# rhmes/point-cloud-compression

Hardware: AMD Instinct MI355X
Metric: points/sec compress+decompress (ModelNet40-shaped 8192 K=256) (higher is better)
Workload: dtype f32 (operands split into two scaled fp16 pieces of 22-23 bits together, three fp16-MFMA products per fp32 product, fp32 accumulate); 1 GPU; IPDAE K=256 d=16 L=7, 8192-pt CAD-like synthetic clouds (configs[1]); distinct_clouds_per_gpu=1024, points_per_cloud=8192, patches_per_cloud=64, octree_mode=reference, weights=seeded random, matmul=f16x2

## Files before the change

### point-cloud-compression_amd/csrc/encoder_fused_h2.hip

```cpp
#include <math.h>
#include <stdlib.h>

#include "blobs.h"
#include "common.h"
#include "mfma_chain.h"

#ifndef FH_CHUNK
#define FH_CHUNK PN_H2_CHUNK
#endif
static_assert(FH_CHUNK % 8 == 0 && ((PN_H2_STREAM_FRAGS + FH_CHUNK - 1) / FH_CHUNK) * FH_CHUNK <= PN_H2_STREAM_CHUNKS * PN_H2_CHUNK, "the padded stream must cover the last chunk");
#ifndef FH_SA_MG
#define FH_SA_MG 2
#endif
#ifndef FH_NB
#define FH_NB 2
#endif
#ifndef FH_MG
#define FH_MG 2
#endif
#ifndef FH_READER
#define FH_READER 1
#endif
#ifndef FH_FIFO
#define FH_FIFO 8
#endif
#ifndef FH_FIFO2
#define FH_FIFO2 8
#endif
#define FH_STAGE_STRIDE 132
#define FH_STAGE_WAVE (16 * FH_STAGE_STRIDE)

__host__ __device__ inline size_t fh_region_bytes()
{
    const size_t ring = (size_t)FH_NB * FH_CHUNK * 1024, stage = (size_t)8 * FH_STAGE_WAVE * 4;
    return ring > stage ? ring : stage;
}
__host__ __device__ inline size_t fh_lds_bytes(int K)
{
    return (size_t)(ENC_H2_SA_W1_FRAGS + ENC_H2_SA_W2_FRAGS) * 1024 + (64 + 128 + ENC_H2_PN_BIAS_FLOATS) * 4 + (size_t)K * 12 + (size_t)K * 32 +
           fh_region_bytes() + 8 * 16 * 4 + 32 + 16;
}

template <bool NT2>
__global__ __launch_bounds__(512, 1) void sa_pn_forward_h2_kernel(const float *__restrict__ x, int npatches, int K, const float *__restrict__ blob,
                                                                  const float *__restrict__ h2, int d, float spread, float half_spread,
                                                                  float *__restrict__ latent_raw, float *__restrict__ latent,
                                                                  float *__restrict__ latent_q, const unsigned char *__restrict__ nbr_tab,
                                                                  const int *__restrict__ uniq, const int *__restrict__ n_uniq)
{
    extern __shared__ __attribute__((aligned(16))) unsigned char smem[];
    f32x4 *sw1 = (f32x4 *)smem;
    f32x4 *sw2 = sw1 + ENC_H2_SA_W1_FRAGS * 64;
    float *sb1 = (float *)(sw2 + ENC_H2_SA_W2_FRAGS * 64);
    float *sb2 = sb1 + 64;
    float *spb = sb2 + 128;
    float *sx = spb + ENC_H2_PN_BIAS_FLOATS;
    unsigned short *nbr16 = (unsigned short *)(sx + 3 * K);
    unsigned char *region = (unsigned char *)(nbr16 + 16 * K);
    f32x4 *swt = (f32x4 *)region;
    float *stage_all = (float *)region;
    float (*smax)[16] = (float (*)[16])(region + fh_region_bytes());
    int *sa_next = (int *)(region + fh_region_bytes() + 8 * 16 * 4);
    unsigned *srmax = (unsigned *)(sa_next + 8);

    const int ntiles = K >> 4;
    const int wu = __builtin_amdgcn_readfirstlane((int)threadIdx.x >> 6);
    auto fresh_lane = []() {
        int l = (int)__builtin_amdgcn_mbcnt_hi(~0u, __builtin_amdgcn_mbcnt_lo(~0u, 0u));
        asm volatile("" : "+v"(l));
        return l;
    };
    auto meta = [&](int i) { return __uint_as_float(__builtin_amdgcn_readfirstlane(__float_as_uint(opaque_uniform(h2)[ENC_H2_META + i]))); };
    {
        const int tid0 = threadIdx.x;
        const f32x4 *gw = (const f32x4 *)(h2 + ENC_H2_SA_W);
        for (int i = tid0; i < (ENC_H2_SA_W1_FRAGS + ENC_H2_SA_W2_FRAGS) * 64; i += 512) sw1[i] = gw[i];
        if (tid0 == 0) *srmax = 0u;
    }
    __syncthreads();
  const int nlist = uniq ? *n_uniq : npatches;
  for (int slot = blockIdx.x; slot < nlist; slot += gridDim.x) {
    const size_t P = uniq ? (size_t)uniq[slot] : (size_t)slot;
    const int lane = fresh_lane(), tid = wu * 64 + lane;
    const float *xp = x + P * (size_t)K * 3;
    {
        unsigned m = 0u;
        for (int i = tid; i < 3 * K; i += 512) m = max(m, __float_as_uint(xp[i]) & 0x7FFFFFFFu);
#pragma unroll
        for (int o = 32; o >= 1; o >>= 1) m = max(m, (unsigned)__shfl_xor((int)m, o));
        if (lane == 0) atomicMax(srmax, m);
    }
    if (tid < 8) sa_next[tid] = 0;
    {
        const uint4 *tab = (const uint4 *)nbr_tab + P * (size_t)K * (K <= 256 ? 1 : 2);
        if (K <= 256) {
            for (int i = tid; i < K; i += 512) {
                const uint4 v = tab[i];
                const unsigned b[4] = {v.x, v.y, v.z, v.w};
                unsigned wd[8];
#pragma unroll
                for (int q = 0; q < 4; ++q) {
                    wd[2 * q] = (b[q] & 0xFFu) | ((b[q] & 0xFF00u) << 8);
                    wd[2 * q + 1] = ((b[q] >> 16) & 0xFFu) | ((b[q] >> 8) & 0xFF0000u);
                }
                ((uint4 *)nbr16)[2 * i] = make_uint4(wd[0], wd[1], wd[2], wd[3]);
                ((uint4 *)nbr16)[2 * i + 1] = make_uint4(wd[4], wd[5], wd[6], wd[7]);
            }
        } else {
            for (int i = tid; i < 2 * K; i += 512) ((uint4 *)nbr16)[i] = tab[i];
        }
    }
    __syncthreads();
    const int rexp = (int)((unsigned)__builtin_amdgcn_readfirstlane((int)*srmax) >> 23) - 127;
    const float s = rexp >= 0 ? __uint_as_float((unsigned)(126 - rexp) << 23) : 1.0f;
    const float inv_s = rexp >= 0 ? __uint_as_float((unsigned)(128 + rexp) << 23) : 1.0f;
    for (int i = tid; i < 3 * K; i += 512) sx[i] = xp[i] * s;
    if (tid < 64) sb1[tid] = h2[ENC_H2_SA_B1 + tid] * s;
    if (tid < 128) sb2[tid] = h2[ENC_H2_SA_B2 + tid] * s;
    for (int i = tid; i < ENC_H2_PN_BIAS_FLOATS; i += 512) spb[i] = h2[ENC_H2_PN_B0 + i] * s;
    __syncthreads();
    if (tid == 0) *srmax = 0u;

    const f32x4 zero4 = {0.f, 0.f, 0.f, 0.f};
    if (lane < 16) smax[wu][lane] = -INFINITY;

    auto sa_and_handover = [&](int it, f16x8 (&i0p)[1][5][2], bool &valid) {
        const int tile = it * 8 + wu;
        valid = tile < ntiles;
        const int p0 = (valid ? tile : 0) * 16;
        int lane = fresh_lane();
        int g = lane >> 4, n = lane & 15;
        const float rho0 = meta(H2E_RHO0), rho1 = meta(H2E_RHO1), inv2 = meta(H2E_INV2);
        const float w0a = blob[ENC_SA_W0B0 + 4 * n + g], w0b = blob[ENC_SA_W0B0 + 4 * (16 + n) + g];

        const int pass_base = it * 128;
        const int units = ((K - pass_base < 128 ? K - pass_base : 128) + 1) >> 1;
        for (;;) {
            int unit = 0;
            if (lane == 0) unit = atomicAdd(&sa_next[it & 7], 1);
            unit = __builtin_amdgcn_readfirstlane(unit);
            if (unit >= units) break;
            const int i0 = pass_base + 2 * unit;
            f32x4 h0[2][2];
#pragma unroll
            for (int nt = 0; nt < 2; ++nt) {
                const int i = i0 + nt;
                const int j = nbr16[i * 16 + n];
                const float rel = g < 3 ? __fsub_rn(sx[3 * j + g], sx[3 * i + g]) : s;
                h0[nt][0] = relu4(mfma16(w0a, rel, zero4));
                h0[nt][1] = relu4(mfma16(w0b, rel, zero4));
            }
            f32x4 a1[2][4];
#pragma unroll
            for (int mt = 0; mt < 4; ++mt) a1[0][mt] = a1[1][mt] = *(const f32x4 *)(sb1 + 16 * mt + 4 * g);
            f32x4 a2[2][8];
#pragma unroll
            for (int mt = 0; mt < 8; ++mt) a2[0][mt] = a2[1][mt] = zero4;
            f16x8 i1[2][1][2];
#pragma unroll
            for (int nt = 0; nt < 2; ++nt) h2_split8(h0[nt][0], h0[nt][1], rho0, i1[nt][0]);
            dense_h2<1, 4, 2>(sw1, lane, i1, a1);
            f16x8 i2[2][2][2];
#pragma unroll
            for (int nt = 0; nt < 2; ++nt)
#pragma unroll
                for (int t = 0; t < 2; ++t) h2_split8(relu4(a1[nt][2 * t]), relu4(a1[nt][2 * t + 1]), rho1, i2[nt][t]);
            dense_h2<2, 8, 2, true, FH_SA_MG>(sw2, lane, i2, a2);
#pragma unroll
            for (int nt = 0; nt < 2; ++nt) {
                float mx[2];
                max16_of_8_transposed_tiles(a2[nt], mx);
#pragma unroll
                for (int s2 = 0; s2 < 2; ++s2) {
                    const int ch = 16 * (2 * g + s2) + n;
                    stage_all[(i0 + nt - pass_base) * FH_STAGE_STRIDE + ch] = fmaxf(__fadd_rn(__fmul_rn(mx[s2], inv2), sb2[ch]), 0.f);
                }
            }
        }

        __syncthreads();
        lane = fresh_lane();
        g = lane >> 4; n = lane & 15;
        {
            const float rho_in = meta(H2E_RHO_IN);
            f32x4 in[9];
            const float *stage_t = stage_all + (valid ? p0 - pass_base : 0) * FH_STAGE_STRIDE;
#pragma unroll
            for (int kt = 0; kt < 8; ++kt) in[kt] = *(const f32x4 *)(stage_t + n * FH_STAGE_STRIDE + 16 * kt + 4 * g);
            const int p = p0 + n;
            in[8][0] = g == 0 ? sx[3 * p] : 0.f;
            in[8][1] = g == 0 ? sx[3 * p + 1] : 0.f;
            in[8][2] = g == 0 ? sx[3 * p + 2] : 0.f;
            in[8][3] = 0.f;
#pragma unroll
            for (int t = 0; t < 4; ++t) h2_split8(in[2 * t], in[2 * t + 1], rho_in, i0p[0][t]);
            h2_split8(in[8], zero4, rho_in, i0p[0][4]);
        }
        __syncthreads();
    };

    const int passes = (ntiles + 7) / 8;
    if constexpr (!NT2) {
      for (int it = 0; it < passes; ++it) {
        f16x8 i0p[1][5][2];
        bool valid;
        sa_and_handover(it, i0p, valid);
        const int lane = fresh_lane();
        const int g = lane >> 4, n = lane & 15;
        const float rho_p1 = meta(H2E_RHO_P1), rho_p2 = meta(H2E_RHO_P2), rho_p3 = meta(H2E_RHO_P3);
        WStreamT<FH_CHUNK, FH_NB, 8> ws{opaque_uniform(h2) + ENC_H2_PN_STREAM, swt, (PN_H2_STREAM_FRAGS + FH_CHUNK - 1) / FH_CHUNK, lane, wu, false};
        ws.prologue();
        int f = 0;
#if FH_READER
        H2Reader<FH_FIFO, PN_H2_STREAM_FRAGS, decltype(ws)> rd(ws);
        rd.start();
#define FH_DENSE(KT, MT, in, acc) dense_h2_rd<KT, MT, 1>(rd, f, in, acc)
#else
#define FH_DENSE(KT, MT, in, acc) dense_h2_stream<KT, MT, 1, decltype(ws), FH_MG>(ws, f, in, acc)
#endif
        f32x4 a0[1][8];
#pragma unroll
        for (int mt = 0; mt < 8; ++mt) a0[0][mt] = *(const f32x4 *)(spb + 16 * mt + 4 * g);
        FH_DENSE(5, 8, i0p, a0);
        f16x8 p1[8][1][1][2];
        {
            f32x4 a1p[1][16];
            f16x8 i1p[1][4][2];
#pragma unroll
            for (int t = 0; t < 4; ++t) h2_split8(relu4(a0[0][2 * t]), relu4(a0[0][2 * t + 1]), rho_p1, i1p[0][t]);
#pragma unroll
            for (int mt = 0; mt < 16; ++mt) a1p[0][mt] = *(const f32x4 *)(spb + 128 + 16 * mt + 4 * g);
            FH_DENSE(4, 16, i1p, a1p);
#pragma unroll
            for (int kt = 0; kt < 8; ++kt) h2_split8(relu4(a1p[0][2 * kt]), relu4(a1p[0][2 * kt + 1]), rho_p2, p1[kt][0][0]);
        }
        f32x4 a3[1][1];
        a3[0][0] = *(const f32x4 *)(spb + 128 + 256 + 512 + 4 * g);
#pragma clang loop unroll(full)
        for (int h = 0; h < 2; ++h) {
            f32x4 a2p[1][16];
#pragma unroll
            for (int mt = 0; mt < 16; ++mt) a2p[0][mt] = *(const f32x4 *)(spb + 128 + 256 + 16 * (16 * h + mt) + 4 * g);
#pragma clang loop unroll(full)
            for (int kt = 0; kt < 8; ++kt) FH_DENSE(1, 16, p1[kt], a2p);
#pragma clang loop unroll(full)
            for (int kt = 0; kt < 8; ++kt) {
                f16x8 pl[1][1][2];
                h2_split8(relu4(a2p[0][2 * kt]), relu4(a2p[0][2 * kt + 1]), rho_p3, pl[0][0]);
                FH_DENSE(1, 1, pl, a3);
            }
        }
#undef FH_DENSE
        ws.drain();
        if (valid) {
#pragma unroll
            for (int r = 0; r < 4; ++r) {
                const float v = row16_max(a3[0][0][r]);
                if (n == 0) smax[wu][4 * g + r] = fmaxf(smax[wu][4 * g + r], v);
            }
        }
        __syncthreads();
      }
    } else {
      for (int rnd = 0; rnd < passes / 2; ++rnd) {
        f16x8 i1p[2][4][2];
#pragma clang loop unroll(full)
        for (int hf = 0; hf < 2; ++hf) {
            f16x8 i0p[1][5][2];
            bool valid;
            sa_and_handover(2 * rnd + hf, i0p, valid);
            const int lane = fresh_lane();
            const int g = lane >> 4;
            const float rho_p1 = meta(H2E_RHO_P1);
            WStreamT<FH_CHUNK, FH_NB, 8> ws0{opaque_uniform(h2) + ENC_H2_PN_STREAM2, swt, PN_H2_S2_L0_FRAGS / FH_CHUNK, lane, wu, false};
            ws0.prologue();
            int f = 0;
            H2Reader<FH_FIFO2, 80, decltype(ws0)> rd0(ws0);
            rd0.start();
            f32x4 a0[1][8];
#pragma unroll
            for (int mt = 0; mt < 8; ++mt) a0[0][mt] = *(const f32x4 *)(spb + 16 * mt + 4 * g);
            dense_h2_rd<5, 8, 1>(rd0, f, i0p, a0);
#pragma unroll
            for (int t = 0; t < 4; ++t) h2_split8(relu4(a0[0][2 * t]), relu4(a0[0][2 * t + 1]), rho_p1, i1p[hf][t]);
            ws0.drain();
            __syncthreads();
        }
        const int lane = fresh_lane();
        const int g = lane >> 4, n = lane & 15;
        const float rho_p2 = meta(H2E_RHO_P2), rho_p3 = meta(H2E_RHO_P3);
        WStreamT<FH_CHUNK, FH_NB, 8> ws{opaque_uniform(h2) + ENC_H2_PN_STREAM2 + (size_t)PN_H2_S2_L0_FRAGS * 256, swt, PN_H2_S2_MAIN_FRAGS / FH_CHUNK, lane, wu, false};
        ws.prologue();
        int f = 0;
        H2Reader<FH_FIFO2, PN_H2_S2_MAIN_FRAGS, decltype(ws)> rd(ws);
        rd.start();
        f16x8 p1[8][2][1][2];
        {
            f32x4 a1p[2][16];
#pragma unroll
            for (int mt = 0; mt < 16; ++mt) a1p[0][mt] = a1p[1][mt] = *(const f32x4 *)(spb + 128 + 16 * mt + 4 * g);
            dense_h2_rd<4, 16, 2>(rd, f, i1p, a1p);
#pragma unroll
            for (int kt = 0; kt < 8; ++kt)
#pragma unroll
                for (int nt = 0; nt < 2; ++nt) h2_split8(relu4(a1p[nt][2 * kt]), relu4(a1p[nt][2 * kt + 1]), rho_p2, p1[kt][nt][0]);
        }
        f32x4 a3[2][1];
        a3[0][0] = a3[1][0] = *(const f32x4 *)(spb + 128 + 256 + 512 + 4 * g);
#pragma clang loop unroll(full)
        for (int e = 0; e < 8; ++e) {
            f32x4 a2p[2][4];
#pragma unroll
            for (int mt = 0; mt < 4; ++mt) a2p[0][mt] = a2p[1][mt] = *(const f32x4 *)(spb + 128 + 256 + 16 * (4 * e + mt) + 4 * g);
#pragma clang loop unroll(full)
            for (int kt = 0; kt < 8; ++kt) dense_h2_rd<1, 4, 2>(rd, f, p1[kt], a2p);
#pragma clang loop unroll(full)
            for (int t = 0; t < 2; ++t) {
                f16x8 pl[2][1][2];
#pragma unroll
                for (int nt = 0; nt < 2; ++nt) h2_split8(relu4(a2p[nt][2 * t]), relu4(a2p[nt][2 * t + 1]), rho_p3, pl[nt][0]);
                dense_h2_rd<1, 1, 2>(rd, f, pl, a3);
            }
        }
        ws.drain();
#pragma unroll
        for (int nt = 0; nt < 2; ++nt)
#pragma unroll
            for (int r = 0; r < 4; ++r) {
                const float v = row16_max(a3[nt][0][r]);
                if (n == 0) smax[wu][4 * g + r] = fmaxf(smax[wu][4 * g + r], v);
            }
        __syncthreads();
      }
    }
    __syncthreads();
    if (tid < 16 && tid < d) {
        const float inv_out = meta(H2E_INV_OUT);
        float m = smax[0][tid];
#pragma unroll
        for (int k8 = 1; k8 < 8; ++k8) m = fmaxf(m, smax[k8][tid]);
        m = __fmul_rn(__fmul_rn(m, inv_out), inv_s);
        const float sg = 1.0f / (1.0f + expf(-m));
        const float y = __fsub_rn(__fmul_rn(sg, spread), half_spread);
        latent_raw[P * d + tid] = m;
        latent[P * d + tid] = y;
        latent_q[P * d + tid] = rintf(y);
    }
    __syncthreads();
  }
}

extern "C" int pccx_ae_encode_h2_fused_ok(int K)
{
    return (K >= 16 && K <= 1024 && K % 16 == 0 && fh_lds_bytes(K) <= (size_t)160 * 1024) ? 1 : 0;
}

extern "C" size_t pccx_ae_encode_h2_workspace_bytes(int P, int K) { return pccx_patch_knn16_bytes(P, K); }
extern "C" int pccx_ae_encode_h2_tables(const float *patches, int P, int K, const float *enc_blob, const float *h2_blob, int d, int L,
                                        float *latent_raw, float *latent, float *latent_q, const void *workspace, void *stream);

extern "C" int pccx_ae_encode_h2_ws(const float *patches, int P, int K, const float *enc_blob, const float *h2_blob, int d, int L,
                                    float *latent_raw, float *latent, float *latent_q, void *workspace, void *stream)
{
    if (P == 0) return PCCX_OK;
    PCCX_CHECK_ARG(patches && workspace, "pccx_ae_encode_h2_ws: null pointer");
    PCCX_CHECK_ARG(P >= 0 && pccx_ae_encode_h2_fused_ok(K), "pccx_ae_encode_h2_ws: K=%d does not fit the fused kernel (pccx_ae_encode_h2_fused_ok)", K);
    const int rc = pccx_patch_knn16(patches, P, K, workspace, stream);
    if (rc != PCCX_OK) return rc;
    return pccx_ae_encode_h2_tables(patches, P, K, enc_blob, h2_blob, d, L, latent_raw, latent, latent_q, workspace, stream);
}

extern "C" int pccx_ae_encode_h2_tables_list(const float *patches, int P, int K, const float *enc_blob, const float *h2_blob, int d, int L,
                                             float *latent_raw, float *latent, float *latent_q, const void *workspace, const int32_t *uniq,
                                             const int32_t *n_uniq, void *stream)
{
    if (P == 0) return PCCX_OK;
    PCCX_CHECK_ARG(patches && enc_blob && h2_blob && latent_raw && latent && latent_q && workspace, "pccx_ae_encode_h2_tables: null pointer");
    PCCX_CHECK_ARG(P >= 0 && pccx_ae_encode_h2_fused_ok(K), "pccx_ae_encode_h2_tables: K=%d does not fit the fused kernel (pccx_ae_encode_h2_fused_ok)", K);
    PCCX_CHECK_ARG(d >= 1 && d <= 16 && L >= 1, "pccx_ae_encode_h2_tables: unsupported d=%d L=%d", d, L);
    PCCX_CHECK_ARG(!uniq == !n_uniq, "pccx_ae_encode_h2_tables_list: uniq and n_uniq come together");
    PCCX_CHECK_ARG(((uintptr_t)workspace & 15) == 0, "pccx_ae_encode_h2_tables: the tables must be 16-byte aligned");
    const float spread = (float)((double)L - 0.2);
    const float half = (float)(((double)L - 0.2) / 2);
    const int grid = P < 2048 ? P : 2048;
    const char *e = getenv("PCCX_ENC_H2_NT");
    const bool nt2 = K % 256 == 0 && !(e && atoi(e) == 1);
    if (nt2) {
        PCCX_CHECK_HIP(hipFuncSetAttribute(reinterpret_cast<const void *>(&sa_pn_forward_h2_kernel<true>), hipFuncAttributeMaxDynamicSharedMemorySize, 160 * 1024));
        hipLaunchKernelGGL(sa_pn_forward_h2_kernel<true>, dim3(grid), dim3(512), fh_lds_bytes(K), (hipStream_t)stream, patches, P, K, enc_blob, h2_blob, d,
                           spread, half, latent_raw, latent, latent_q, (const unsigned char *)workspace, uniq, n_uniq);
    } else {
        PCCX_CHECK_HIP(hipFuncSetAttribute(reinterpret_cast<const void *>(&sa_pn_forward_h2_kernel<false>), hipFuncAttributeMaxDynamicSharedMemorySize, 160 * 1024));
        hipLaunchKernelGGL(sa_pn_forward_h2_kernel<false>, dim3(grid), dim3(512), fh_lds_bytes(K), (hipStream_t)stream, patches, P, K, enc_blob, h2_blob, d,
                           spread, half, latent_raw, latent, latent_q, (const unsigned char *)workspace, uniq, n_uniq);
    }
    PCCX_CHECK_LAUNCH();
    return PCCX_OK;
}

extern "C" int pccx_ae_encode_h2_tables(const float *patches, int P, int K, const float *enc_blob, const float *h2_blob, int d, int L,
                                        float *latent_raw, float *latent, float *latent_q, const void *workspace, void *stream)
{
    return pccx_ae_encode_h2_tables_list(patches, P, K, enc_blob, h2_blob, d, L, latent_raw, latent, latent_q, workspace, nullptr, nullptr, stream);
}
```

Before: 1.116 billion points/s.

## Prefetch next patch's points and neighbor table into LDS during current patch

```diff
diff --git a/point-cloud-compression_amd/csrc/encoder_fused_h2.hip b/point-cloud-compression_amd/csrc/encoder_fused_h2.hip
--- a/point-cloud-compression_amd/csrc/encoder_fused_h2.hip
+++ b/point-cloud-compression_amd/csrc/encoder_fused_h2.hip
@@ -40,8 +40,64 @@
     return (size_t)(ENC_H2_SA_W1_FRAGS + ENC_H2_SA_W2_FRAGS) * 1024 + (64 + 128 + ENC_H2_PN_BIAS_FLOATS) * 4 + (size_t)K * 12 + (size_t)K * 32 +
            fh_region_bytes() + 8 * 16 * 4 + 32 + 16;
 }
-
-template <bool NT2>
+#define FH_IDX_WINDOW 32
+#define FH_FETCH_WAVES 4
+#define FH_BIAS_FLOATS (64 + 128 + ENC_H2_PN_BIAS_FLOATS)
+__host__ __device__ inline size_t fh_tab_bytes(int K) { return (size_t)K * (K <= 256 ? 16 : 32); }
+__host__ __device__ inline size_t fh_lds_bytes_pf(int K)
+{
+    return fh_lds_bytes(K) + (size_t)K * 12 + fh_tab_bytes(K) + FH_BIAS_FLOATS * 4 + (FH_IDX_WINDOW + 4) * 4;
+}
+
+#ifdef FH_STAMPS
+#define FH_STAMP_WGS 4096
+__device__ unsigned long long fh_stamps[FH_STAMP_WGS * 8];
+extern "C" __attribute__((visibility("default"))) int pccx_debug_fh_stamps(unsigned long long *out, int wgs, int reset)
+{
+    if (wgs < 0 || wgs > FH_STAMP_WGS) return -1;
+    if (out && hipMemcpyFromSymbol(out, HIP_SYMBOL(fh_stamps), sizeof(unsigned long long) * 8 * wgs) != hipSuccess) return -1;
+    if (reset) {
+        void *p = nullptr;
+        if (hipGetSymbolAddress(&p, HIP_SYMBOL(fh_stamps)) != hipSuccess || pccx_zero_async(p, sizeof(unsigned long long) * 8 * FH_STAMP_WGS, nullptr) != hipSuccess ||
+            hipDeviceSynchronize() != hipSuccess)
+            return -1;
+    }
+    return 0;
+}
+__device__ __forceinline__ unsigned long long fh_now()
+{
+    unsigned long long t;
+    __builtin_amdgcn_sched_barrier(0);
+    asm volatile("s_memrealtime %0\n\ts_waitcnt lgkmcnt(0)" : "=s"(t)::"memory");
+    __builtin_amdgcn_sched_barrier(0);
+    return t;
+}
+#define FH_STAMP_EARLY 30000
+#define FH_STAMP_ENTRY() [[maybe_unused]] unsigned long long fh_setup = 0, fh_rest = 0, fh_n = 0, fh_early = 0, fh_ne = 0; const unsigned long long fh_t0 = fh_now()
+#define FH_STAMP_PROLOGUE() const unsigned long long fh_t1 = fh_now()
+#define FH_STAMP_TOP() const unsigned long long fh_ta = fh_now()
+#define FH_STAMP_SETUP() const unsigned long long fh_tb = fh_now(); fh_setup += fh_tb - fh_ta
+#define FH_STAMP_PATCH()                                                                                                               \
+    {                                                                                                                                  \
+        const unsigned long long dt = fh_now() - fh_tb;                                                                                \
+        fh_rest += dt, ++fh_n;                                                                                                         \
+        if (fh_tb - fh_t0 < FH_STAMP_EARLY) fh_early += dt, ++fh_ne;                                                                   \
+    }
+#define FH_STAMP_END()                                                                                                                 \
+    if (threadIdx.x == 0 && blockIdx.x < FH_STAMP_WGS) {                                                                               \
+        unsigned long long *o = fh_stamps + 8 * blockIdx.x;                                                                            \
+        o[0] = fh_t0, o[1] = fh_t1, o[2] += fh_setup, o[3] += fh_rest, o[4] = fh_now(), o[5] += fh_n, o[6] += fh_early, o[7] += fh_ne; \
+    }
+#else
+#define FH_STAMP_ENTRY()
+#define FH_STAMP_PROLOGUE()
+#define FH_STAMP_TOP()
+#define FH_STAMP_SETUP()
+#define FH_STAMP_PATCH()
+#define FH_STAMP_END()
+#endif
+
+template <bool NT2, bool PF>
 __global__ __launch_bounds__(512, 1) void sa_pn_forward_h2_kernel(const float *__restrict__ x, int npatches, int K, const float *__restrict__ blob,
                                                                   const float *__restrict__ h2, int d, float spread, float half_spread,
                                                                   float *__restrict__ latent_raw, float *__restrict__ latent,
@@ -62,6 +118,11 @@
     float (*smax)[16] = (float (*)[16])(region + fh_region_bytes());
     int *sa_next = (int *)(region + fh_region_bytes() + 8 * 16 * 4);
     unsigned *srmax = (unsigned *)(sa_next + 8);
+    float *px = (float *)(smem + fh_lds_bytes(K));
+    unsigned char *ptab = (unsigned char *)(px + 3 * K);
+    float *sbraw = (float *)(ptab + fh_tab_bytes(K));
+    int *sidx = (int *)(sbraw + FH_BIAS_FLOATS);
+    int *sexit = (int *)(srmax + 1);
 
     const int ntiles = K >> 4;
     const int wu = __builtin_amdgcn_readfirstlane((int)threadIdx.x >> 6);
@@ -71,18 +132,47 @@
         return l;
     };
     auto meta = [&](int i) { return __uint_as_float(__builtin_amdgcn_readfirstlane(__float_as_uint(opaque_uniform(h2)[ENC_H2_META + i]))); };
+    auto fetch_patch = [&](int Pn, int part, int nparts) {
+        const int l16 = fresh_lane() * 16;
+        const char *gx = (const char *)(x + (size_t)Pn * K * 3), *gt = (const char *)nbr_tab + (size_t)Pn * fh_tab_bytes(K);
+        const int nx = 12 * K, nt = (int)fh_tab_bytes(K), bx = (nx + 1023) >> 10, bt = (nt + 1023) >> 10;
+        for (int b = part; b < bx + bt; b += nparts) {
+            const int o = (b < bx ? b : b - bx) << 10;
+            if (b < bx) {
+                if (o + l16 < nx) __builtin_amdgcn_global_load_lds((const void *)(gx + o + l16), (lds_u32 *)(uintptr_t)((char *)px + o), 16, 0, 0);
+            } else {
+                if (o + l16 < nt) __builtin_amdgcn_global_load_lds((const void *)(gt + o + l16), (lds_u32 *)(uintptr_t)(ptab + o), 16, 0, 0);
+            }
+        }
+    };
+    const int nlist = uniq ? *n_uniq : npatches;
+    FH_STAMP_ENTRY();
+    if constexpr (PF) {
+        if ((int)blockIdx.x < nlist) fetch_patch(uniq ? uniq[blockIdx.x] : (int)blockIdx.x, wu, 8);
+        for (int i = threadIdx.x; i < FH_BIAS_FLOATS; i += 512) sbraw[i] = h2[ENC_H2_SA_B1 + i];
+    }
     {
         const int tid0 = threadIdx.x;
         const f32x4 *gw = (const f32x4 *)(h2 + ENC_H2_SA_W);
         for (int i = tid0; i < (ENC_H2_SA_W1_FRAGS + ENC_H2_SA_W2_FRAGS) * 64; i += 512) sw1[i] = gw[i];
         if (tid0 == 0) *srmax = 0u;
     }
+    if constexpr (PF) asm volatile("s_waitcnt vmcnt(0)" ::: "memory");
     __syncthreads();
-  const int nlist = uniq ? *n_uniq : npatches;
-  for (int slot = blockIdx.x; slot < nlist; slot += gridDim.x) {
-    const size_t P = uniq ? (size_t)uniq[slot] : (size_t)slot;
+    FH_STAMP_PROLOGUE();
+  for (int slot = blockIdx.x, iter = 0; slot < nlist; slot += gridDim.x, ++iter) {
+    FH_STAMP_TOP();
     const int lane = fresh_lane(), tid = wu * 64 + lane;
-    const float *xp = x + P * (size_t)K * 3;
+    size_t P = 0;
+    if constexpr (!PF) P = uniq ? (size_t)uniq[slot] : (size_t)slot;
+    const float *xp = PF ? px : x + P * (size_t)K * 3;
+    if constexpr (PF) {
+        if ((iter & (FH_IDX_WINDOW - 1)) == 0 && tid <= FH_IDX_WINDOW) {
+            const long long sl = (long long)slot + (long long)tid * gridDim.x;
+            sidx[tid] = sl < nlist ? (uniq ? uniq[sl] : (int)sl) : -1;
+        }
+        if (tid == 8) *sexit = 0;
+    }
     {
         unsigned m = 0u;
         for (int i = tid; i < 3 * K; i += 512) m = max(m, __float_as_uint(xp[i]) & 0x7FFFFFFFu);
@@ -92,7 +182,7 @@
     }
     if (tid < 8) sa_next[tid] = 0;
     {
-        const uint4 *tab = (const uint4 *)nbr_tab + P * (size_t)K * (K <= 256 ? 1 : 2);
+        const uint4 *tab = PF ? (const uint4 *)ptab : (const uint4 *)nbr_tab + P * (size_t)K * (K <= 256 ? 1 : 2);
         if (K <= 256) {
             for (int i = tid; i < K; i += 512) {
                 const uint4 v = tab[i];
@@ -111,14 +201,20 @@
         }
     }
     __syncthreads();
+    if constexpr (PF) P = (size_t)__builtin_amdgcn_readfirstlane(sidx[iter & (FH_IDX_WINDOW - 1)]);
     const int rexp = (int)((unsigned)__builtin_amdgcn_readfirstlane((int)*srmax) >> 23) - 127;
     const float s = rexp >= 0 ? __uint_as_float((unsigned)(126 - rexp) << 23) : 1.0f;
     const float inv_s = rexp >= 0 ? __uint_as_float((unsigned)(128 + rexp) << 23) : 1.0f;
     for (int i = tid; i < 3 * K; i += 512) sx[i] = xp[i] * s;
-    if (tid < 64) sb1[tid] = h2[ENC_H2_SA_B1 + tid] * s;
-    if (tid < 128) sb2[tid] = h2[ENC_H2_SA_B2 + tid] * s;
-    for (int i = tid; i < ENC_H2_PN_BIAS_FLOATS; i += 512) spb[i] = h2[ENC_H2_PN_B0 + i] * s;
+    if constexpr (PF) {
+        for (int i = tid; i < FH_BIAS_FLOATS; i += 512) sb1[i] = sbraw[i] * s;
+    } else {
+        if (tid < 64) sb1[tid] = h2[ENC_H2_SA_B1 + tid] * s;
+        if (tid < 128) sb2[tid] = h2[ENC_H2_SA_B2 + tid] * s;
+        for (int i = tid; i < ENC_H2_PN_BIAS_FLOATS; i += 512) spb[i] = h2[ENC_H2_PN_B0 + i] * s;
+    }
     __syncthreads();
+    FH_STAMP_SETUP();
     if (tid == 0) *srmax = 0u;
 
     const f32x4 zero4 = {0.f, 0.f, 0.f, 0.f};
@@ -178,6 +274,16 @@
             }
         }
 
+        if constexpr (PF) {
+            if (it == 0) {
+                int rank = 0;
+                if (lane == 0) rank = atomicAdd(sexit, 1);
+                rank = __builtin_amdgcn_readfirstlane(rank);
+                const int Pn = __builtin_amdgcn_readfirstlane(sidx[(iter & (FH_IDX_WINDOW - 1)) + 1]);
+                if (rank < FH_FETCH_WAVES && Pn >= 0) fetch_patch(Pn, rank, FH_FETCH_WAVES);
+                asm volatile("s_waitcnt vmcnt(0)" ::: "memory");
+            }
+        }
         __syncthreads();
         lane = fresh_lane();
         g = lane >> 4; n = lane & 15;
@@ -347,7 +453,9 @@
         latent_q[P * d + tid] = rintf(y);
     }
     __syncthreads();
+    FH_STAMP_PATCH();
   }
+    FH_STAMP_END();
 }
 
 extern "C" int pccx_ae_encode_h2_fused_ok(int K)
@@ -368,6 +476,19 @@
     const int rc = pccx_patch_knn16(patches, P, K, workspace, stream);
     if (rc != PCCX_OK) return rc;
     return pccx_ae_encode_h2_tables(patches, P, K, enc_blob, h2_blob, d, L, latent_raw, latent, latent_q, workspace, stream);
+}
+
+static int fh_compute_units()
+{
+    static int cus[64];
+    int dev = 0;
+    if (hipGetDevice(&dev) != hipSuccess || dev < 0 || dev >= 64) return 0;
+    if (cus[dev] == 0) {
+        int n = 0;
+        if (hipDeviceGetAttribute(&n, hipDeviceAttributeMultiprocessorCount, dev) != hipSuccess) return 0;
+        cus[dev] = n;
+    }
+    return cus[dev];
 }
 
 extern "C" int pccx_ae_encode_h2_tables_list(const float *patches, int P, int K, const float *enc_blob, const float *h2_blob, int d, int L,
@@ -382,18 +503,30 @@
     PCCX_CHECK_ARG(((uintptr_t)workspace & 15) == 0, "pccx_ae_encode_h2_tables: the tables must be 16-byte aligned");
     const float spread = (float)((double)L - 0.2);
     const float half = (float)(((double)L - 0.2) / 2);
-    const int grid = P < 2048 ? P : 2048;
+    int grid = P < 2048 ? P : 2048;
+    if (uniq) {
+        const int cus = fh_compute_units();
+        PCCX_CHECK_ARG(cus > 0, "pccx_ae_encode_h2_tables_list: cannot read the device's compute-unit count");
+        grid = P < cus ? P : cus;
+    }
+    if (const char *g = getenv("PCCX_ENC_H2_GRID")) {
+        const int n = atoi(g);
+        PCCX_CHECK_ARG(n >= 1 && n <= 65536, "PCCX_ENC_H2_GRID=%s: expected 1 .. 65536", g);
+        grid = n;
+    }
     const char *e = getenv("PCCX_ENC_H2_NT");
     const bool nt2 = K % 256 == 0 && !(e && atoi(e) == 1);
-    if (nt2) {
-        PCCX_CHECK_HIP(hipFuncSetAttribute(reinterpret_cast<const void *>(&sa_pn_forward_h2_kernel<true>), hipFuncAttributeMaxDynamicSharedMemorySize, 160 * 1024));
-        hipLaunchKernelGGL(sa_pn_forward_h2_kernel<true>, dim3(grid), dim3(512), fh_lds_bytes(K), (hipStream_t)stream, patches, P, K, enc_blob, h2_blob, d,
-                           spread, half, latent_raw, latent, latent_q, (const unsigned char *)workspace, uniq, n_uniq);
-    } else {
-        PCCX_CHECK_HIP(hipFuncSetAttribute(reinterpret_cast<const void *>(&sa_pn_forward_h2_kernel<false>), hipFuncAttributeMaxDynamicSharedMemorySize, 160 * 1024));
-        hipLaunchKernelGGL(sa_pn_forward_h2_kernel<false>, dim3(grid), dim3(512), fh_lds_bytes(K), (hipStream_t)stream, patches, P, K, enc_blob, h2_blob, d,
-                           spread, half, latent_raw, latent, latent_q, (const unsigned char *)workspace, uniq, n_uniq);
-    }
+    const char *pe = getenv("PCCX_ENC_H2_PREFETCH");
+    const bool pf = fh_lds_bytes_pf(K) <= (size_t)160 * 1024 && ((uintptr_t)patches & 15) == 0 && !(pe && atoi(pe) == 0);
+    auto launch = [&](auto kernel, size_t lds) {
+        if (hipFuncSetAttribute(reinterpret_cast<const void *>(kernel), hipFuncAttributeMaxDynamicSharedMemorySize, 160 * 1024) != hipSuccess) return false;
+        hipLaunchKernelGGL(kernel, dim3(grid), dim3(512), lds, (hipStream_t)stream, patches, P, K, enc_blob, h2_blob, d, spread, half, latent_raw,
+                           latent, latent_q, (const unsigned char *)workspace, uniq, n_uniq);
+        return true;
+    };
+    const bool ok = nt2 ? (pf ? launch(&sa_pn_forward_h2_kernel<true, true>, fh_lds_bytes_pf(K)) : launch(&sa_pn_forward_h2_kernel<true, false>, fh_lds_bytes(K)))
+                        : (pf ? launch(&sa_pn_forward_h2_kernel<false, true>, fh_lds_bytes_pf(K)) : launch(&sa_pn_forward_h2_kernel<false, false>, fh_lds_bytes(K)));
+    PCCX_CHECK_ARG(ok, "pccx_ae_encode_h2_tables: hipFuncSetAttribute(MaxDynamicSharedMemorySize) failed");
     PCCX_CHECK_LAUNCH();
     return PCCX_OK;
 }
```

Result: slower. 1.093 billion points/s (-2.0%).
